# peterdavidfagan/mujoco_robot_environments

Measured on AMD Instinct MI355X. Metric: env steps/sec (whole node), RearrangementEnv batch=4096 at 1/2/4/8 MI355X, higher is better.
Workload: dtype f32

## Files before the change

### mujoco_robot_environments_amd/csrc/mre_api.cpp

```cpp
#include <hip/hip_runtime.h>

#include <cmath>
#include <cstdio>
#include <cstdlib>
#include <cstring>
#include <string>
#include <algorithm>
#include <vector>

#include "mre_env.h"
#include "mre_labels.h"
#include "mre_launch.h"
#include "mre_model.h"
#include "mre_records.h"

using namespace mre;

static thread_local std::string g_err;
int mre::fail(int code, const std::string& msg) {
  g_err = msg;
  return code;
}

extern "C" const char* mre_last_error(void) { return g_err.c_str(); }
// ... 29 lines not shown
  HIPCHK(hipMalloc(&e->sv_converged, N));
  HIPCHK(hipHostMalloc((void**)&e->h_launch_info, mre_env::RING * N * 16, hipHostMallocMapped | hipHostMallocCoherent));
  HIPCHK(hipHostGetDevicePointer((void**)&e->d_launch_info, e->h_launch_info, 0));
  memset(e->h_launch_info, 0xFF, mre_env::RING * N * 16);
  HIPCHK(hipHostMalloc((void**)&e->h_info_last, N * 16, hipHostMallocDefault));
  memset(e->h_info_last, 0xFF, N * 16);
  HIPCHK(hipHostMalloc((void**)&e->h_large_stage, mre_env::NSTAGE * N, hipHostMallocMapped | hipHostMallocCoherent));
  HIPCHK(hipHostGetDevicePointer((void**)&e->d_large_stage, e->h_large_stage, 0));
  memset(e->h_large_stage, 0, mre_env::NSTAGE * N);
  HIPCHK(hipMalloc(&e->d_pending, N));
  HIPCHK(hipMemsetAsync(e->d_pending, 0, N, e->stream));
  HIPCHK(hipMemsetAsync(e->d_large, 0, N, e->stream));
  e->h_large.assign(N, 0); e->h_rerun.assign(N, 0);
  { int rc = sched_create(e); if (rc) return rc; }
  if (const char* fb = getenv("MRE_NO_FALLBACK")) e->fallback = atoi(fb) == 0;
  if (const char* fl = getenv("MRE_FORCE_LARGE")) {
    if (atoi(fl) != 0) {
      e->h_large.assign(N, 1); e->n_large = num_envs;
      HIPCHK(hipMemsetAsync(e->d_large, 1, N, e->stream));
    }
  }
  HIPCHK(hipMemsetAsync(e->status, 0, N * 4, e->stream)); HIPCHK(hipMemsetAsync(e->stats, 0, N * 16, e->stream));
  HIPCHK(hipMemsetAsync(e->grip_closed, 0, N, e->stream)); HIPCHK(hipMemsetAsync(e->osc_target, 0, N * 64, e->stream));
  HIPCHK(hipMemsetAsync(e->sites, 0, N * 64, e->stream));
  std::vector<int> np(N, NPROP);
  std::vector<float> ps(N * NPROP * 3, 0.0155f);
  HIPCHK(hipMemcpy(e->nprops, np.data(), N * 4, hipMemcpyHostToDevice));
  HIPCHK(hipMemcpy(e->prop_size, ps.data(), ps.size() * 4, hipMemcpyHostToDevice));
  e->osc = OscConfig{350.f, 20.f, 500.f, 100.f, 200.f, 30.f, {0.f, -0.785f, 0.f, -2.356f, 0.f, 1.571f, 0.785f},
                     5e-3f, 68e-3f, 0};
// ... 574 lines not shown
  if (!e || !w) return fail(MRE_ERR_ARG, "null");
  DRAIN(e);
  return copy_out(e, w, e->qacc_ws, (size_t)e->N * NVP * 4);
}
extern "C" int mre_set_ctrl(mre_env* e, const float* ctrl) {
  if (!e || !ctrl) return fail(MRE_ERR_ARG, "null");
  DRAIN(e);
  return copy_in(e, e->ctrl, ctrl, (size_t)e->N * NU * 4);
}

static void fill_args(mre_env* e, StepArgs& a) {
  memset(&a, 0, sizeof(a));
  a.M = e->dM; a.N = e->N; a.seq_stride = e->N;
  a.qpos = e->qpos; a.qvel = e->qvel; a.qacc_ws = e->qacc_ws; a.ctrl = e->ctrl; a.qfine = e->qfine;
  a.nprops = e->nprops; a.prop_size = e->prop_size;
  a.control_steps = 1; a.mode = CTRL_HELD;
  a.osc = e->d_osc_env ? e->d_osc_env : e->d_osc; a.osc_stride = e->d_osc_env ? 1 : 0;
  a.osc_target = e->osc_target; a.grip_closed = e->grip_closed;
  a.sites = e->sites; a.status = e->status; a.stats = e->stats; a.nstep = e->nstep;
  a.env_order = e->use_order ? e->order : (e->have_auto_order ? e->auto_order : nullptr);
  a.trace = e->trace; a.trace_nenv = e->trace_nenv; a.trace_max = e->trace_max; a.trace_base = e->trace_pos;
}

extern "C" int mre_step(mre_env* e, int nsubsteps, unsigned flags) {
  if (!e || nsubsteps < 0) return fail(MRE_ERR_ARG, "mre_step: bad argument");
  StepArgs a;
  fill_args(e, a);
  a.nsteps = nsubsteps; a.flags = flags;
  if (nsubsteps > 0) a.sites = nullptr;
  int rc = launch_step(e, a);
  if (rc) return rc;
  if (e->trace) e->trace_pos += nsubsteps;
  return MRE_OK;
}

extern "C" int mre_rollout_ticks(mre_env* e, const float* ctrl_seq, int nticks, int control_steps, unsigned flags,
                                 int ticks_per_launch) {
  if (!e || !ctrl_seq || nticks < 0 || control_steps < 1) return fail(MRE_ERR_ARG, "mre_rollout: bad argument");
  if (!is_device_ptr(ctrl_seq)) return fail(MRE_ERR_ARG, "mre_rollout: ctrl_seq must be a device pointer");
  int per = (ticks_per_launch <= 0 || ticks_per_launch > nticks) ? nticks : ticks_per_launch;
  bool allow_queue = ticks_per_launch >= 2;
  if (ticks_per_launch <= 0 && policy::queue_fits(e->queue_ok, e->queue_waves, e->N) && nticks >= 2) {
    if (policy::window_wants_queue(nticks, e->queue_min_ticks, e->tick_tail_valid, e->tick_tail, e->queue_tail_min)) {
// ... 9 lines not shown
    const size_t n = (size_t)nticks * (size_t)e->N * NU;
    if (n > e->seq_cap) {
      DRAIN_PENDING(e);
      for (float*& p : e->seq_copy) { if (p) HIPCHK(hipFree(p)); p = nullptr; HIPCHK(hipMalloc(&p, n * 4)); }
      e->seq_cap = n;
    }
    float* dst = e->seq_copy[e->seq_calls++ % (unsigned)(mre_env::RING + 1)];
    HIPCHK(hipMemcpyAsync(dst, ctrl_seq, n * 4, hipMemcpyDeviceToDevice, e->stream));
    src = dst;
  }
  for (int t0 = 0; t0 < nticks || (nticks == 0 && t0 == 0); t0 += per) {
    const int nt = nticks - t0 < per ? nticks - t0 : per;
    StepArgs a;
    fill_args(e, a);
    a.nsteps = nt * control_steps; a.control_steps = control_steps; a.mode = CTRL_SEQ;
    a.ctrl_seq = src + (size_t)t0 * (size_t)e->N * NU; a.flags = flags;
    a.sites = nullptr;
    int rc = launch_step(e, a, false, true, allow_queue);
    if (rc) return rc;
    if (e->trace) e->trace_pos += a.nsteps;
    if (nticks == 0) break;
  }
  return MRE_OK;
}

extern "C" int mre_rollout(mre_env* e, const float* ctrl_seq, int nticks, int control_steps, unsigned flags) {
  return mre_rollout_ticks(e, ctrl_seq, nticks, control_steps, flags, 0);
}

extern "C" int mre_set_trace(mre_env* e, float* out, int nenv, int max_steps) {
  if (!e) return fail(MRE_ERR_ARG, "null handle");
// ... 152 lines not shown
    if (t0 + n < nticks) a.flags |= F_CONV_OPEN;
    int rc = launch_step(e, a, false, queue || !(converged_out != nullptr && chunk >= nticks), queue);
    if (rc) return rc;
    if (e->trace) e->trace_pos += a.nsteps;
    t0 += n;
  } while (t0 < nticks);
  if (converged_out) { DRAIN(e); return copy_out(e, converged_out, e->converged, (size_t)e->N); }
  return MRE_OK;
}

extern "C" int mre_osc_compute(mre_env* e, float* tau, float* grip) {
  if (!e) return fail(MRE_ERR_ARG, "null handle");
  DRAIN(e);
  StepArgs a;
  fill_args(e, a);
  a.nsteps = 0; a.control_steps = 1; a.mode = CTRL_OSC; a.flags = F_OSC_EVAL; a.trace = nullptr;
  HIPCHK(hipSetDevice(e->device));
  step_kernels(e->solver).step(&a, e->stream);
  HIPCHK(hipGetLastError());
  const size_t N = (size_t)e->N;
  std::vector<float> h(N * NU);
  int rc = copy_out(e, h.data(), e->ctrl, N * NU * 4);
  if (rc) return rc;
  std::vector<float> ht(N * 7), hg(N);
  for (size_t i = 0; i < N; i++) {
    for (int k = 0; k < 7; k++) ht[i * 7 + k] = h[i * NU + k];
    hg[i] = h[i * NU + 7];
  }
  if (tau) { rc = copy_out(e, tau, ht.data(), N * 7 * 4); if (rc) return rc; }
  if (grip) { rc = copy_out(e, grip, hg.data(), N * 4); if (rc) return rc; }
  return MRE_OK;
}

static int search_buffers(mre_env* e) {
  if (e->ps_attempts) return MRE_OK;
  const size_t N = (size_t)e->N;
  HIPCHK(hipMalloc(&e->ps_attempts, N * 4)); HIPCHK(hipMalloc(&e->ps_prop, N * 4));
  HIPCHK(hipMalloc(&e->ps_tick, N * 4)); HIPCHK(hipMalloc(&e->ps_which, N * 4));
  HIPCHK(hipMalloc(&e->ps_bounds, N * 6 * 8)); HIPCHK(hipMalloc(&e->ps_pose, N * 7 * 8));
  HIPCHK(hipMalloc(&e->ps_zones, N * NPROP * 4 * 8)); HIPCHK(hipMalloc(&e->ps_pick, N * 7 * 8));
  return MRE_OK;
}
static void fill_search(mre_env* e, SearchArgs& sa) {
  memset(&sa, 0, sizeof(sa));
  sa.M = e->dM; sa.N = e->N; sa.qpos = e->qpos; sa.qfine = e->qfine; sa.nprops = e->nprops; sa.prop_size = e->prop_size;
  sa.env_ids = e->d_env_ids; sa.env_id_offset = e->env_id_offset;
  sa.attempts = e->ps_attempts; sa.fixed_prop = -1;
}

static int detect_contacts(mre_env* e, const uint8_t* dmask, bool full = false, bool active_only = false) {
  const size_t N = (size_t)e->N, row = 1 + 3 * CONTACT_EXPORT;
  if (!e->contacts) HIPCHK(hipMalloc(&e->contacts, N * row * 4));
  if (full && !e->contacts_full) HIPCHK(hipMalloc(&e->contacts_full, N * CONTACT_EXPORT * 12 * 4));
  StepArgs a;
  fill_args(e, a);
  a.nsteps = 0; a.flags = F_DETECT | (active_only ? F_DETECT_ACTIVE : 0u); a.trace = nullptr; a.env_mask = dmask;
  a.contacts = e->contacts; a.contacts_full = full ? e->contacts_full : nullptr;
  a.sites = nullptr; a.geoms = nullptr;
  step_kernels(e->solver).step(&a, e->stream);
  HIPCHK(hipGetLastError());
  return MRE_OK;
}

extern "C" int mre_get_contacts(mre_env* e, int32_t* count, float* contacts) {
  if (!e || !count || !contacts) return fail(MRE_ERR_ARG, "mre_get_contacts: null");
  DRAIN(e);
  HIPCHK(hipSetDevice(e->device));
  int rc = detect_contacts(e, nullptr);
  if (rc) return rc;
  const size_t N = (size_t)e->N, row = 1 + 3 * CONTACT_EXPORT;
  std::vector<float> h(N * row);
// ... 97 lines not shown
      mre_launch_pose_search(&sa, e->stream);
      HIPCHK(hipGetLastError());
      if ((rc = copy_out(e, att.data(), e->ps_attempts, N * 4))) return rc;
      bool dropped = false;
      for (size_t i = 0; i < N; i++)
        if (todo[i] && p < np[i] && att[i] <= 0) { failed[i] = 1; todo[i] = 0; dropped = true; }
      if (dropped && (rc = copy_in(e, e->mask, todo.data(), N))) return rc;
    }
    HIPCHK(hipStreamSynchronize(e->stream));
    if (settle_steps <= 0) break;
    StepArgs a;
    fill_args(e, a);
    a.trace = nullptr;
    a.nsteps = (int)std::lround(2.0 / e->hM.opt_rec.timestep);
    if (a.nsteps < settle_steps) a.nsteps = settle_steps;
    a.flags = F_FREEZE_ROBOT | F_SETTLE_EXIT; a.env_mask = e->mask;
    a.settle_steps = e->settle_steps; a.min_settle_steps = settle_steps;
    const bool prof = e->profiling;
    e->profiling = false;
    rc = launch_step(e, a, true);
    e->profiling = prof;
    if (rc) return rc;
    if ((rc = copy_out(e, hs.data(), e->settle_steps, N * 4))) return rc;
    if (getenv("MRE_DEBUG_PLACE")) {
      int nt = 0, ns = 0;
      for (size_t i = 0; i < N; i++) if (todo[i]) { nt++; ns += hs[i] >= 0; }
      fprintf(stderr, "mre_place_props round %d: %d envs placed, %d settled\n", round, nt, ns);
    }
    int settled_now = 0;
    for (size_t i = 0; i < N; i++) {
      if (!todo[i]) continue;
// ... 159 lines not shown
```

### mujoco_robot_environments_amd/csrc/mre_collide.h

```cpp
#pragma once
#include "mre_math.h"

namespace mre {

constexpr int COLL_BUF = 48;
MRE_DEV float* cand_xyz(float* buf, int k) { return buf + 24 + 3 * k; }
MRE_DEV float& cand_dist(float* buf, int k) { return buf[3 * k + 2]; }

MRE_DEV float sel3(const float* v, int i) {
  const float w0 = i == 0 ? 1.f : 0.f, w1 = i == 1 ? 1.f : 0.f, w2 = i == 2 ? 1.f : 0.f;
  return w0 * v[0] + w1 * v[1] + w2 * v[2];
}
MRE_DEV void row3(float* o, const float (*m)[3], int i) {
  const float w0 = i == 0 ? 1.f : 0.f, w1 = i == 1 ? 1.f : 0.f, w2 = i == 2 ? 1.f : 0.f;
  o[0] = w0 * m[0][0] + w1 * m[1][0] + w2 * m[2][0];
  o[1] = w0 * m[0][1] + w1 * m[1][1] + w2 * m[2][1];
  o[2] = w0 * m[0][2] + w1 * m[1][2] + w2 * m[2][2];
}

MRE_DEV int clip_poly(float* p, float* q, int n, float sx, float sy) {
  float* src = p;
  float* dst = q;
  for (int e = 0; e < 4; e++) {
    const int ax = e >> 1;
// ... 10 lines not shown
      if (da <= 0 && nq < 8) { dst[3 * nq] = a0; dst[3 * nq + 1] = a1; dst[3 * nq + 2] = a2; nq++; }
      if ((da <= 0) != (db <= 0) && nq < 8) {
        const float t = da / (da - db);
        dst[3 * nq] = a0 + t * (b0 - a0); dst[3 * nq + 1] = a1 + t * (b1 - a1); dst[3 * nq + 2] = a2 + t * (b2 - a2);
        nq++;
      }
      a0 = b0; a1 = b1; a2 = b2;
    }
    n = nq;
    if (n == 0) return 0;
    float* t = src; src = dst; dst = t;
  }
  return n;
}

MRE_DEV int box_box(const float* p1, const float* R1, const float* s1, const float* p2,
                    const float* R2, const float* s2, float margin, float* normal, float* buf) {
  float* poly = buf;
  float* qbuf = buf + 24;
  float A[3][3], B[3][3], dv[3], Cm[3][3], aC[3][3];
#pragma unroll
  for (int i = 0; i < 3; i++)
#pragma unroll
    for (int k = 0; k < 3; k++) { A[i][k] = R1[3 * k + i]; B[i][k] = R2[3 * k + i]; }
  v3sub(dv, p2, p1);
#pragma unroll
  for (int i = 0; i < 3; i++)
#pragma unroll
    for (int j = 0; j < 3; j++) { Cm[i][j] = v3dot(A[i], B[j]); aC[i][j] = fabsf(Cm[i][j]); }
  float tA[3], tB[3];
#pragma unroll
  for (int i = 0; i < 3; i++) { tA[i] = v3dot(dv, A[i]); tB[i] = v3dot(dv, B[i]); }
// ... 92 lines not shown
    const float dd = fabsf(v3dot(nr, Ai[k]));
    if (dd > bestd) { bestd = dd; kk = k; }
  }
  const int ku = (kk + 1) % 3, kv = (kk + 2) % 3, au = (a + 1) % 3, av = (a + 2) % 3;
  float Aik[3], Aiu[3], Aiv[3], Aru[3], Arv[3];
  row3(Aik, Ai, kk); row3(Aiu, Ai, ku); row3(Aiv, Ai, kv);
  row3(Aru, Ar, au); row3(Arv, Ar, av);
  const float sik = sel3(siv3, kk), siu = sel3(siv3, ku), siv = sel3(siv3, kv);
  const float sra = sel3(srv3, a), sru = sel3(srv3, au), srv = sel3(srv3, av);
  const float isg = v3dot(nr, Aik) >= 0 ? -1.0f : 1.0f;
  float ci[3], cr[3];
  v3copy(ci, pi);
  v3addscl(ci, Aik, isg * sik);
  v3copy(cr, pr);
  v3addscl(cr, nr, sra);
#pragma unroll
  for (int v = 0; v < 4; v++) {
    const float su = (v == 0 || v == 3) ? 1.0f : -1.0f;
    const float sv = (v < 2) ? 1.0f : -1.0f;
    float w[3];
    v3copy(w, ci);
    v3addscl(w, Aiu, su * siu);
    v3addscl(w, Aiv, sv * siv);
    v3sub(w, w, cr);
    poly[3 * v] = v3dot(w, Aru);
    poly[3 * v + 1] = v3dot(w, Arv);
    poly[3 * v + 2] = v3dot(w, nr);
  }
  const int n = clip_poly(poly, qbuf, 4, sru, srv);
  int nc = 0;
  for (int v = 0; v < n; v++) {
    const float x = poly[3 * v], y = poly[3 * v + 1], dep = poly[3 * v + 2];
    if (dep > margin) continue;
    float* cx = cand_xyz(buf, nc);
    cx[0] = cr[0] + x * Aru[0] + y * Arv[0] + 0.5f * dep * nr[0];
    cx[1] = cr[1] + x * Aru[1] + y * Arv[1] + 0.5f * dep * nr[1];
    cx[2] = cr[2] + x * Aru[2] + y * Arv[2] + 0.5f * dep * nr[2];
    cand_dist(buf, nc) = dep;
    nc++;
  }
  return nc;
}

// ... 132 lines not shown
```

### mujoco_robot_environments_amd/csrc/mre_dev.h

```cpp
#pragma once
#include <stdint.h>

namespace mre {

constexpr int NB = 20;
constexpr int NRB = 16;
constexpr int GRIP_BODY0 = 8;
constexpr int NV = 39;
constexpr int NRV = 15;
constexpr int NQ = 43;
constexpr int NQP = 44;
constexpr int TRACE_W = 88;
constexpr int TRACE_QVEL = 48;
constexpr int NVP = 40;
constexpr int NU = 8;
constexpr int QFINE = 32;
constexpr int QFINE_ROW = 96;
constexpr int QFINE_CUBE_Q = 32;
constexpr int QFINE_CUBE_V = 60;
static_assert(QFINE_CUBE_Q + 7 * 4 == QFINE_CUBE_V && QFINE_CUBE_V + 6 * 4 <= QFINE_ROW, "qfine row layout");
constexpr int NPROP = 4;
constexpr int NG = 20;
constexpr int PROP_GEOM0 = 12;
constexpr int NPAIR = 128;
// ... 138 lines not shown
  MEntryRec m_rec[NMR];
  RowRec row_rec[NROWREC];
  EqRec eq_rec[NEQ];
  SiteRec site_rec[NSITE];
  OptRec opt_rec;
};

struct OscConfig {
  float kp_pos, kd_pos, kp_ori, kd_ori, kp_null, kd_null;
  float null_q[7];
  float pos_thresh, ori_thresh;
  int pinv_always;
};

enum StepFlags : unsigned { F_NO_CONSTRAINTS = 1u, F_FREEZE_ROBOT = 2u, F_CONV_CONTINUE = 4u, F_CONV_OPEN = 8u,
                            F_OSC_EVAL = 16u, F_DETECT = 32u, F_SETTLE_EXIT = 64u, F_DETECT_ACTIVE = 128u };
enum CtrlMode : int { CTRL_HELD = 0, CTRL_SEQ = 1, CTRL_OSC = 2 };

struct StepArgs {
  const DevModel* M;
  int N;
  float* qpos;
  float* qvel;
  float* qacc_ws;
  float* qfine;
  float* ctrl;
  const float* ctrl_seq;
  int seq_stride;
  const int* nprops;
  const float* prop_size;
  int nsteps, control_steps, mode;
// ... 53 lines not shown
  unsigned long long seed;
  const int* prop;
  int fixed_prop;
  const double* bounds;
  double shared_bounds[6];
  const int* tick_base;
  long long tick0;
  int max_attempts;
  int yaw_mode;
  double fixed_quat[4];
  float max_dist;
  int commit;
  float* qfine;
  double* pose;
  int* attempts;
};

constexpr int DYN_W = 128;
constexpr int DYN_JAC = 0, DYN_MASS = 42, DYN_BIAS = 91, DYN_POS = 98, DYN_QUAT = 101, DYN_QPOS = 105, DYN_QVEL = 112,
              DYN_PAD = 119;
struct DynArgs {
  const DevModel* M;
  int N;
  const float* qpos;
  const float* qvel;
  const float* qfine;
  const int* nprops;
  const float* prop_size;
  int site;
  float* out;
// ... 38 lines not shown
```

### mujoco_robot_environments_amd/csrc/mre_env.h

```cpp
#pragma once
#include <hip/hip_runtime.h>

#include <string>
#include <utility>
#include <vector>

#include "../../include/mre.h"
#include "mre_dev.h"
#include "mre_policy.h"

#define HIPCHK(x)                                                                       \
  do {                                                                                  \
    hipError_t e_ = (x);                                                                \
    if (e_ != hipSuccess)                                                               \
      return mre::fail(MRE_ERR_HIP, std::string(#x) + ": " + hipGetErrorString(e_));    \
  } while (0)

struct mre_env {
  int N = 0, device = 0;
  hipStream_t stream = nullptr;
  mre::DevModel* dM = nullptr;
  mre::DevModel hM;
  int solver = MRE_SOLVER_PGS;
  float *qpos = nullptr, *qvel = nullptr, *qacc_ws = nullptr, *ctrl = nullptr;
// ... 17 lines not shown
  uint8_t* prop_rgb = nullptr;
  float geom_rgb[mre::NG][3];
  float* trace = nullptr;
  int trace_nenv = 0, trace_max = 0, trace_pos = 0;
  long long env_id_offset = 0;
  std::vector<long long> env_ids;
  int* order = nullptr;
  bool use_order = false;
  int* auto_order = nullptr;
  int* h_auto_order = nullptr;
  bool have_auto_order = false;
  bool profiling = false;
  std::vector<std::pair<hipEvent_t, hipEvent_t>> events;
  size_t events_used = 0;
  bool fallback = true;
  bool large_only = false;
  bool compact_only = false;
  hipStream_t stream2 = nullptr;
  hipEvent_t ev_fork = nullptr, ev_join = nullptr, ev_order = nullptr;
  uint8_t *d_large = nullptr, *mask_r = nullptr;
  float *sv_qpos = nullptr, *sv_qvel = nullptr, *sv_qacc_ws = nullptr, *sv_ctrl = nullptr, *sv_qfine = nullptr;
  uint32_t* sv_status = nullptr;
  uint8_t* sv_converged = nullptr;
  float* contacts = nullptr;
  float* contacts_full = nullptr;
  int* settle_steps = nullptr;
  int* h_launch_info = nullptr;
  int* d_launch_info = nullptr;
  int* h_info_last = nullptr;
  uint8_t* d_pending = nullptr;
// ... 86 lines not shown
```

### mujoco_robot_environments_amd/csrc/mre_kernels.hip

```cpp
#include <hip/hip_runtime.h>

#include "mre_dev.h"
#include "mre_math.h"
#include "mre_collide.h"

namespace mre {
using ModelP = MRE_MODEL_PTR(DevModel);
#if defined(MRE_PHASE_STAMPS) && MRE_PHASE_STAMPS >= 4
__shared__ unsigned long long dbg_acc[4];
#endif

struct OscSm {
  float J[6][7], M[7][7], MiJt[7][6], Li[6][6], Lam[6][6], V[6][6], Jbar[7][6];
  float ep[3], eo[3], F[6], LF[6], tn[7], Jbt[6], xd[6], w[6];
};

struct alignas(8) Blk {
  uint16_t row0;
  uint8_t type, nrows;
  uint8_t rslot;
  uint8_t pa, pb;
  uint8_t primary : 4;
  uint8_t bslot : 4;
};
// ... 1382 lines not shown
    crb_mass_matrix(M, s, l);
    MRE_SYNC();
#ifndef MRE_NEWTON
    factor_robot_regs(s.qM, s.qLD, s.qLDinv);
#endif
    MRE_STAMP(15);
    MRE_STAMP(0);

    velocity_stage(M, s, l);
    MRE_SYNC();
    finger_bias(M, s, l);
    MRE_STAMP(1);
    const bool constrained = (a.flags & F_NO_CONSTRAINTS) == 0;
    if (constrained) {

      collide(M, s, l, false);
      MRE_STAMP(2);
      assemble_constraints(M, s, l);
#ifdef MRE_NEWTON
      nw_build_lists(s, l);
#else
      solve_robot_rows(s, l);
      assemble_blocks(M, s, l);
#endif
      MRE_STAMP(3);
      hw_ncon = max(hw_ncon, s.ncon); hw_nefc = max(hw_nefc, s.nefc);
      hw_nrrow = max(hw_nrrow, s.nrrow); hw_npp = max(hw_npp, s.npp);
    }

    if (a.mode == CTRL_SEQ && (step % a.control_steps) == 0) {
      const int tick = step / a.control_steps;
// ... 85 lines not shown
    else a.nstep[env] += steps_done;
  }
  if (a.nsteps == 0 && (a.flags & F_OSC_EVAL) != 0 && a.mode == CTRL_OSC) {
    position_stage(M, s, l);
    gripper_local(M, s, l);
    crb_mass_matrix(M, s, l);
    MRE_SYNC();
    velocity_stage(M, s, l);
    MRE_SYNC();
    osc_compute(M, s, osc, oscp, s.osc_tgt, l);
    if (l == 0) s.ctrl[NU - 1] = grip_cmd;
    MRE_SYNC();
  }
  if (a.nsteps == 0 && (a.flags & F_DETECT) != 0 && a.contacts != nullptr) {
    position_stage(M, s, l);
    collide(M, s, l, (a.flags & F_DETECT_ACTIVE) == 0);
    float* o = a.contacts + (size_t)env * (1 + 3 * CONTACT_EXPORT);
    const int n = s.ncon < CONTACT_EXPORT ? s.ncon : CONTACT_EXPORT;
    if (l == 0) o[0] = s.overflow ? -(float)s.ncon : (float)s.ncon;
    if (l < n) {
      const int pr = s.con_pair[l];
      o[1 + 3 * l] = (float)M->pair_g1[pr]; o[2 + 3 * l] = (float)M->pair_g2[pr]; o[3 + 3 * l] = s.con_dist[l];
      if (a.contacts_full != nullptr) {
        float* f = a.contacts_full + ((size_t)env * CONTACT_EXPORT + l) * 12;
        for (int k = 0; k < 3; k++) f[k] = s.con_pos[l][k];
        for (int k = 0; k < 9; k++) f[3 + k] = s.con_frame[l][k];
      }
    }
    MRE_SYNC();
    if (l == 0) s.overflow = 0;
  }
// ... 237 lines not shown
      float xq[4] = {(float)pose[3], (float)pose[4], (float)pose[5], (float)pose[6]};
      qnormalize(xq);
      for (int k = 0; k < 3; k++) s.xpos[body][k] = (float)pose[k];
      for (int k = 0; k < 4; k++) s.xquat[body][k] = xq[k];
      q2mat(s.xmat[body], xq);
    }
    MRE_SYNC();
    bool hit = false;
    if (pr >= 0) {
      const int g1 = M->pair_g1[pr], g2 = M->pair_g2[pr];
      float p1[3], R1[9], s1[3], rb1, p2[3], R2[9], s2[3], rb2, normal[3] = {0.f, 0.f, 1.f}, df[3];
      geom_pose(M, s, g1, p1, R1, s1, &rb1);
      geom_pose(M, s, g2, p2, R2, s2, &rb2);
      const float inc = M->pair_margin[pr];
      int n = 0;
      v3sub(df, p2, p1);
      if (M->geom_type[g1] == 0) {
        float nn[3] = {R1[2], R1[5], R1[8]};
        if (v3dot(df, nn) - rb2 <= inc) n = plane_box(p1, R1, p2, R2, s2, inc, normal, buf);
      } else {
        const float r = rb1 + rb2 + inc;
        if (v3dot(df, df) <= r * r) n = box_box(p1, R1, s1, p2, R2, s2, inc, normal, buf);
      }
      for (int c = 0; c < n; c++) {
        const float d = cand_dist(buf, c);
        if (d < inc && d <= a.max_dist) hit = true;
      }
    }
    const bool any = __ballot(hit) != 0ull;
    MRE_SYNC();
    if (!any) { used = att + 1; break; }
  }
  if (l == 0) {
    if (a.attempts != nullptr) a.attempts[env] = used;
    if (used > 0) {
      if (a.pose != nullptr) for (int k = 0; k < 7; k++) a.pose[(size_t)env * 7 + k] = pose[k];
      if (a.commit) {
        float* q = a.qpos + (size_t)env * NQP + NRV + 7 * p;
        for (int k = 0; k < 7; k++) q[k] = (float)pose[k];
        if (a.qfine != nullptr) {
          float* ql = a.qfine + (size_t)env * QFINE_ROW;
// ... 207 lines not shown
```

### mujoco_robot_environments_amd/csrc/mre_math.h

```cpp
#pragma once
#include <hip/hip_runtime.h>

#define MRE_DEV __device__ __forceinline__
#if defined(MRE_PHASE_STAMPS) && MRE_PHASE_STAMPS >= 4
#define MRE_DBG_T0() unsigned long long dbg_t_ = __builtin_amdgcn_s_memtime()
#define MRE_DBG_STAMP(SET, K)                                                      \
  do {                                                                             \
    const unsigned long long n_ = __builtin_amdgcn_s_memtime();                    \
    if (MRE_PHASE_STAMPS == (SET) && threadIdx.x == 0) dbg_acc[K] += n_ - dbg_t_;  \
    dbg_t_ = n_;                                                                   \
  } while (0)
#else
#define MRE_DBG_T0() do {} while (0)
#define MRE_DBG_STAMP(SET, K) do {} while (0)
#endif
#define MRE_PHASE_FN __device__ __attribute__((noinline))
#define MRE_SYNC()                                        \
  do {                                                    \
    __builtin_amdgcn_fence(__ATOMIC_ACQ_REL, "wavefront"); \
    __builtin_amdgcn_wave_barrier();                      \
  } while (0)
#if defined(__HIP_DEVICE_COMPILE__)
#define MRE_MODEL_PTR(T) const T __attribute__((address_space(1)))*
#else
#define MRE_MODEL_PTR(T) const T*
#endif

namespace mre {

constexpr float kMinVal = 1e-15f;

MRE_DEV void keep_live(float x) { asm volatile("" ::"v"(x)); }
MRE_DEV void keep_live(int x) { asm volatile("" ::"v"(x)); }

MRE_DEV void v3copy(float* r, const float* a) { r[0] = a[0]; r[1] = a[1]; r[2] = a[2]; }
MRE_DEV void v3zero(float* r) { r[0] = r[1] = r[2] = 0.f; }
MRE_DEV void v3add(float* r, const float* a, const float* b) {
  r[0] = a[0] + b[0]; r[1] = a[1] + b[1]; r[2] = a[2] + b[2];
}
MRE_DEV void v3sub(float* r, const float* a, const float* b) {
  r[0] = a[0] - b[0]; r[1] = a[1] - b[1]; r[2] = a[2] - b[2];
}
MRE_DEV float v3dot(const float* a, const float* b) { return a[0] * b[0] + a[1] * b[1] + a[2] * b[2]; }
MRE_DEV void v3cross(float* r, const float* a, const float* b) {
  float x = a[1] * b[2] - a[2] * b[1], y = a[2] * b[0] - a[0] * b[2], z = a[0] * b[1] - a[1] * b[0];
  r[0] = x; r[1] = y; r[2] = z;
}
MRE_DEV void v3addscl(float* r, const float* a, float s) { r[0] += a[0] * s; r[1] += a[1] * s; r[2] += a[2] * s; }
// ... 90 lines not shown
  v3cross(r, vel, v);
  v3cross(a, vel, v + 3);
  v3cross(b, vel + 3, v);
  v3add(r + 3, a, b);
}
MRE_DEV void cross_force(float* r, const float* vel, const float* f) {
  float a[3], b[3];
  v3cross(a, vel, f);
  v3cross(b, vel + 3, f + 3);
  v3add(r, a, b);
  v3cross(r + 3, vel, f + 3);
}
MRE_DEV float dot6(const float* a, const float* b) {
  return a[0] * b[0] + a[1] * b[1] + a[2] * b[2] + a[3] * b[3] + a[4] * b[4] + a[5] * b[5];
}
template <int CTRL, int ROW_MASK>
MRE_DEV float dpp_add(float v) {
  const int t = __builtin_amdgcn_update_dpp(0, __builtin_bit_cast(int, v), CTRL, ROW_MASK, 0xF, false);
  return v + __builtin_bit_cast(float, t);
}
MRE_DEV float wave_sum(float v) {
  v = dpp_add<0xB1, 0xF>(v);
  v = dpp_add<0x4E, 0xF>(v);
  v = dpp_add<0x141, 0xF>(v);
  v = dpp_add<0x140, 0xF>(v);
  v = dpp_add<0x142, 0xA>(v);
  v = dpp_add<0x143, 0xC>(v);
  return __builtin_bit_cast(float, __builtin_amdgcn_readlane(__builtin_bit_cast(int, v), 63));
}
MRE_DEV void wave_sum3(float& a, float& b, float& c) {
// ... 25 lines not shown
}
template <int CTRL, int ROW_MASK>
MRE_DEV float dpp_max(float v) {
  const int t = __builtin_amdgcn_update_dpp(0, __builtin_bit_cast(int, v), CTRL, ROW_MASK, 0xF, false);
  return fmaxf(v, __builtin_bit_cast(float, t));
}
MRE_DEV float wave_max(float v) {
  v = dpp_max<0xB1, 0xF>(v);
  v = dpp_max<0x4E, 0xF>(v);
  v = dpp_max<0x141, 0xF>(v);
  v = dpp_max<0x140, 0xF>(v);
  v = dpp_max<0x142, 0xA>(v);
  v = dpp_max<0x143, 0xC>(v);
  return __builtin_bit_cast(float, __builtin_amdgcn_readlane(__builtin_bit_cast(int, v), 63));
}
MRE_DEV float clampf(float x, float lo, float hi) { return x < lo ? lo : (x > hi ? hi : x); }

MRE_DEV double rcp64(double x) {
  double r = __builtin_amdgcn_rcp(x);
  r = r * (2.0 - x * r);
  return r * (2.0 - x * r);
}
MRE_DEV double rsq64(double x) {
  double y = __builtin_amdgcn_rsq(x);
  y = y * (1.5 - 0.5 * x * y * y);
  return y * (1.5 - 0.5 * x * y * y);
}


}
```

### mujoco_robot_environments_amd/csrc/mre_solver.h

```cpp
#pragma once

namespace mre {

constexpr int HDR_NONE = 0xFF;
constexpr int BLK_NONE = 0x7F;
constexpr int SCHED_NONE = 0xFF;
constexpr int TAB_OFF = MAXBLK * 5;
constexpr int TAB_ZEROS = 48;
static_assert(TAB_BYTES == 8 * (TAB_OFF + 1) + 4 * TAB_ZEROS, "operand table size");

#ifndef MRE_NEWTON
MRE_DEV void build_schedule(ModelP M, Sm& s);
#endif
MRE_DEV constexpr int cube_pair_bit(int p, int q) {
  const int a = p < q ? p : q, b = p < q ? q : p;
  return a == 0 ? b - 1 : (a == 1 ? b + 1 : 5);
}

MRE_DEV float prop_invM(const Sm& s, int p, int k) {
  return 1.0f / ((k < 3) ? s.prop_mass[p] : s.prop_inertia[p][k - 3]);
}

MRE_DEV void geom_pose(ModelP M, const Sm& s, int g, float* p, float* R, float* size,
                       float* rbound) {
// ... 10 lines not shown
  } else {
    v3copy(size, M->geom_size[g]);
    *rbound = M->geom_rbound[g];
  }
}

MRE_DEV void geom_center(ModelP M, const Sm& s, int g, float* p, float* rbound) {
  const int b = M->geom_body[g];
  float tmp[3];
  m3mulv(tmp, s.xmat[b], M->geom_pos[g]);
  v3add(p, s.xpos[b], tmp);
  const int pid = M->geom_propid[g];
  *rbound = pid >= 0 ? v3norm(s.prop_size[pid]) : M->geom_rbound[g];
}

MRE_PHASE_FN void collide(ModelP M, Sm& s, int l, bool detect) {
  static_assert(offsetof(Sm, hdr) + sizeof(((Sm*)0)->hdr) - offsetof(Sm, JpA) >= sizeof(float) * 64 * COLL_BUF,
                "clip buffers do not fit");
  static_assert(NPAIR <= 256 && sizeof(((Sm*)0)->iscr) >= NPAIR, "survivor list: one byte per pair");
  MRE_DBG_T0();
  float* buf = &s.JpA[0][0] + l * COLL_BUF;
  uint8_t* list = reinterpret_cast<uint8_t*>(s.iscr);
  const unsigned long long lt = (1ull << l) - 1ull;
  int nsurv = 0;
  for (int pass = 0; pass < NPAIR / 64; pass++) {
    const int pr = l + 64 * pass;
    const auto* R = &M->pair_rec[pr];
    const int g1 = R->g1, b1 = R->b1, b2 = R->b2, pid1 = R->pid1, pid2 = R->pid2, type1 = R->type1;
    const float lp1[3] = {R->pos1[0], R->pos1[1], R->pos1[2]}, lp2[3] = {R->pos2[0], R->pos2[1], R->pos2[2]};
    const float mrb1 = R->rb1, mrb2 = R->rb2, margin = R->margin, gap = R->gap;
    const float lq1[4] = {R->quat1[0], R->quat1[1], R->quat1[2], R->quat1[3]};
    bool live = false;
    if (g1 >= 0 && (pid1 < 0 || pid1 < s.nprops) && (pid2 < 0 || pid2 < s.nprops)) {
      const float inc = detect ? margin : margin - gap;
      float p1[3], p2[3], df[3], tmp[3];
      m3mulv(tmp, s.xmat[b1], lp1); v3add(p1, s.xpos[b1], tmp);
// ... 6 lines not shown
        q2mat(R1, q);
        const float nn[3] = {R1[2], R1[5], R1[8]};
        live = v3dot(df, nn) - rb2 <= inc;
      } else {
        const float r = rb1 + rb2 + inc;
        live = v3dot(df, df) <= r * r;
      }
    }
    const unsigned long long m = __ballot(live);
    if (live) list[nsurv + __popcll(m & lt)] = (uint8_t)pr;
    nsurv += __popcll(m);
  }
  if (l == 0) s.ncon = 0;
  MRE_SYNC();
  MRE_DBG_STAMP(6, 0);
  int base = 0;
  for (int c0 = 0; c0 < nsurv; c0 += 64) {
    const int pr = (c0 + l < nsurv) ? list[c0 + l] : -1;
    float normal[3] = {0.f, 0.f, 1.f};
    int n = 0;
    if (pr >= 0) {
      const auto* R = &M->pair_rec[pr];
      const int b1 = R->b1, b2 = R->b2, pid1 = R->pid1, pid2 = R->pid2, type1 = R->type1;
      const float lp1[3] = {R->pos1[0], R->pos1[1], R->pos1[2]}, lp2[3] = {R->pos2[0], R->pos2[1], R->pos2[2]};
      const float lq1[4] = {R->quat1[0], R->quat1[1], R->quat1[2], R->quat1[3]};
      const float lq2[4] = {R->quat2[0], R->quat2[1], R->quat2[2], R->quat2[3]};
      const float ms1[3] = {R->size1[0], R->size1[1], R->size1[2]}, ms2[3] = {R->size2[0], R->size2[1], R->size2[2]};
      const float margin = R->margin, gap = R->gap;
      float p1[3], R1[9], s1[3], p2[3], R2[9], s2[3], tmp[3], q[4];
      m3mulv(tmp, s.xmat[b1], lp1); v3add(p1, s.xpos[b1], tmp);
      qmul(q, s.xquat[b1], lq1); q2mat(R1, q);
      m3mulv(tmp, s.xmat[b2], lp2); v3add(p2, s.xpos[b2], tmp);
      qmul(q, s.xquat[b2], lq2); q2mat(R2, q);
      if (pid1 >= 0) v3copy(s1, s.prop_size[pid1]); else v3copy(s1, ms1);
      if (pid2 >= 0) v3copy(s2, s.prop_size[pid2]); else v3copy(s2, ms2);
      const float inc = detect ? margin : margin - gap;
      MRE_DBG_STAMP(6, 1);
      if ((R->single >> 8) == 2) n = cyl_box(p1, R1, s1, p2, R2, s2[0], s2[2], inc, normal, buf);
      else if (type1 == 0) n = plane_box(p1, R1, p2, R2, s2, inc, normal, buf);
      else n = box_box(p1, R1, s1, p2, R2, s2, inc, normal, buf);
      MRE_DBG_STAMP(6, 2);
      int m = 0;
      for (int c = 0; c < n; c++)
        if (cand_dist(buf, c) < inc) {
          if (m != c) {
            for (int k = 0; k < 3; k++) cand_xyz(buf, m)[k] = cand_xyz(buf, c)[k];
            cand_dist(buf, m) = cand_dist(buf, c);
          }
          m++;
        }
      n = m;
    }
    const bool single = pr >= 0 && n > 1 && (M->pair_rec[pr].single & 0xFF) != 0;
    const int ncand = n;
    if (single) n = 1;
    int off = base, tot = base;
    for (int bit = 0; bit < 4; bit++) {
      const unsigned long long m = __ballot((n >> bit) & 1);
      off += __popcll(m & lt) << bit;
      tot += __popcll(m) << bit;
    }
    if (l == 0) {
      s.ncon = tot < NCON_MAX ? tot : NCON_MAX;
      if (tot > NCON_MAX) s.overflow = 1;
    }
    if (single) {
      const float incw = M->pair_rec[pr].margin - M->pair_rec[pr].gap;
      float wsum = 0.f, px = 0.f, py = 0.f, pz = 0.f, dmin = cand_dist(buf, 0);
      int best = 0;
      for (int c = 0; c < ncand; c++) {
        const float dc = cand_dist(buf, c);
        if (dc < dmin) { dmin = dc; best = c; }
        const float w = incw - dc;
        if (w > 0.f) { wsum += w; px += w * cand_xyz(buf, c)[0]; py += w * cand_xyz(buf, c)[1]; pz += w * cand_xyz(buf, c)[2]; }
      }
      if (wsum > 0.f) { const float iw = 1.0f / wsum; px *= iw; py *= iw; pz *= iw; }
      else { px = cand_xyz(buf, best)[0]; py = cand_xyz(buf, best)[1]; pz = cand_xyz(buf, best)[2]; }
      cand_xyz(buf, 0)[0] = px; cand_xyz(buf, 0)[1] = py; cand_xyz(buf, 0)[2] = pz;
      cand_dist(buf, 0) = dmin;
    }
    if (n > 0) {
      float f[9];
      v3copy(f, normal);
      make_frame(f);
      for (int c = 0; c < n; c++) {
        const int id = off + c;
        if (id >= NCON_MAX) break;
        const float cx0 = cand_xyz(buf, c)[0], cx1 = cand_xyz(buf, c)[1], cx2 = cand_xyz(buf, c)[2];
        s.con_pos[id][0] = cx0; s.con_pos[id][1] = cx1; s.con_pos[id][2] = cx2;
        for (int k = 0; k < 9; k++) s.con_frame[id][k] = f[k];
        s.con_dist[id] = cand_dist(buf, c);
        s.con_pair[id] = (uint8_t)pr;
      }
    }
    MRE_SYNC();
    MRE_DBG_STAMP(6, 3);
    if (tot > NCON_MAX) break;
    base = tot;
  }
}

MRE_DEV float impedance(const float* solimp, float pos, float margin) {
  const float dmin = clampf(solimp[0], 0.0001f, 0.9999f), dmax = clampf(solimp[1], 0.0001f, 0.9999f);
  const float width = fmaxf(solimp[2], kMinVal), mid = clampf(solimp[3], 0.0001f, 0.9999f);
  const float power = fmaxf(solimp[4], 1.0f);
  if (dmin == dmax) return 0.5f * (dmin + dmax);
  const float x = fabsf((pos - margin) / width);
  if (x >= 1.0f) return dmax;
  if (x <= 0.0f) return dmin;
  float y;
  if (power == 1.0f) y = x;
  else if (power == 2.0f) {
    y = (x <= mid) ? x * x / mid : 1.0f - (1.0f - x) * (1.0f - x) / (1.0f - mid);
// ... 855 lines not shown
```

Baseline: 24.58 million.

## Keep unclipped box-box face contacts in registers instead of LDS clip buffer

Adds a fast path in box_box: when all four incident-face vertices already lie inside the reference face rectangle, contact candidates are computed directly into a register struct, skipping the polygon clip and the per-lane shared-memory candidate buffer. Downstream filtering, single-contact averaging and contact emission get matching register-based branches. Collide is split into broad and narrow phase functions, and an env-var flag can force the old clipping path. This adds code size and register pressure, and the extra branches may diverge within a wavefront.

```diff
diff --git a/mujoco_robot_environments_amd/csrc/mre_api.cpp b/mujoco_robot_environments_amd/csrc/mre_api.cpp
--- a/mujoco_robot_environments_amd/csrc/mre_api.cpp
+++ b/mujoco_robot_environments_amd/csrc/mre_api.cpp
@@ -67,6 +67,7 @@
   e->h_large.assign(N, 0); e->h_rerun.assign(N, 0);
   { int rc = sched_create(e); if (rc) return rc; }
   if (const char* fb = getenv("MRE_NO_FALLBACK")) e->fallback = atoi(fb) == 0;
+  if (const char* ng = getenv("MRE_NARROW_GENERIC")) e->base_flags = atoi(ng) != 0 ? F_CLIP_ALWAYS : 0u;
   if (const char* fl = getenv("MRE_FORCE_LARGE")) {
     if (atoi(fl) != 0) {
       e->h_large.assign(N, 1); e->n_large = num_envs;
@@ -671,7 +672,7 @@
   a.M = e->dM; a.N = e->N; a.seq_stride = e->N;
   a.qpos = e->qpos; a.qvel = e->qvel; a.qacc_ws = e->qacc_ws; a.ctrl = e->ctrl; a.qfine = e->qfine;
   a.nprops = e->nprops; a.prop_size = e->prop_size;
-  a.control_steps = 1; a.mode = CTRL_HELD;
+  a.control_steps = 1; a.mode = CTRL_HELD; a.flags = e->base_flags;
   a.osc = e->d_osc_env ? e->d_osc_env : e->d_osc; a.osc_stride = e->d_osc_env ? 1 : 0;
   a.osc_target = e->osc_target; a.grip_closed = e->grip_closed;
   a.sites = e->sites; a.status = e->status; a.stats = e->stats; a.nstep = e->nstep;
@@ -683,7 +684,7 @@
   if (!e || nsubsteps < 0) return fail(MRE_ERR_ARG, "mre_step: bad argument");
   StepArgs a;
   fill_args(e, a);
-  a.nsteps = nsubsteps; a.flags = flags;
+  a.nsteps = nsubsteps; a.flags |= flags;
   if (nsubsteps > 0) a.sites = nullptr;
   int rc = launch_step(e, a);
   if (rc) return rc;
@@ -723,7 +724,7 @@
     StepArgs a;
     fill_args(e, a);
     a.nsteps = nt * control_steps; a.control_steps = control_steps; a.mode = CTRL_SEQ;
-    a.ctrl_seq = src + (size_t)t0 * (size_t)e->N * NU; a.flags = flags;
+    a.ctrl_seq = src + (size_t)t0 * (size_t)e->N * NU; a.flags |= flags;
     a.sites = nullptr;
     int rc = launch_step(e, a, false, true, allow_queue);
     if (rc) return rc;
@@ -906,7 +907,7 @@
   DRAIN(e);
   StepArgs a;
   fill_args(e, a);
-  a.nsteps = 0; a.control_steps = 1; a.mode = CTRL_OSC; a.flags = F_OSC_EVAL; a.trace = nullptr;
+  a.nsteps = 0; a.control_steps = 1; a.mode = CTRL_OSC; a.flags |= F_OSC_EVAL; a.trace = nullptr;
   HIPCHK(hipSetDevice(e->device));
   step_kernels(e->solver).step(&a, e->stream);
   HIPCHK(hipGetLastError());
@@ -937,7 +938,7 @@
   memset(&sa, 0, sizeof(sa));
   sa.M = e->dM; sa.N = e->N; sa.qpos = e->qpos; sa.qfine = e->qfine; sa.nprops = e->nprops; sa.prop_size = e->prop_size;
   sa.env_ids = e->d_env_ids; sa.env_id_offset = e->env_id_offset;
-  sa.attempts = e->ps_attempts; sa.fixed_prop = -1;
+  sa.attempts = e->ps_attempts; sa.fixed_prop = -1; sa.flags = e->base_flags;
 }
 
 static int detect_contacts(mre_env* e, const uint8_t* dmask, bool full = false, bool active_only = false) {
@@ -946,7 +947,7 @@
   if (full && !e->contacts_full) HIPCHK(hipMalloc(&e->contacts_full, N * CONTACT_EXPORT * 12 * 4));
   StepArgs a;
   fill_args(e, a);
-  a.nsteps = 0; a.flags = F_DETECT | (active_only ? F_DETECT_ACTIVE : 0u); a.trace = nullptr; a.env_mask = dmask;
+  a.nsteps = 0; a.flags |= F_DETECT | (active_only ? F_DETECT_ACTIVE : 0u); a.trace = nullptr; a.env_mask = dmask;
   a.contacts = e->contacts; a.contacts_full = full ? e->contacts_full : nullptr;
   a.sites = nullptr; a.geoms = nullptr;
   step_kernels(e->solver).step(&a, e->stream);
@@ -1074,7 +1075,7 @@
     a.trace = nullptr;
     a.nsteps = (int)std::lround(2.0 / e->hM.opt_rec.timestep);
     if (a.nsteps < settle_steps) a.nsteps = settle_steps;
-    a.flags = F_FREEZE_ROBOT | F_SETTLE_EXIT; a.env_mask = e->mask;
+    a.flags |= F_FREEZE_ROBOT | F_SETTLE_EXIT; a.env_mask = e->mask;
     a.settle_steps = e->settle_steps; a.min_settle_steps = settle_steps;
     const bool prof = e->profiling;
     e->profiling = false;
diff --git a/mujoco_robot_environments_amd/csrc/mre_collide.h b/mujoco_robot_environments_amd/csrc/mre_collide.h
--- a/mujoco_robot_environments_amd/csrc/mre_collide.h
+++ b/mujoco_robot_environments_amd/csrc/mre_collide.h
@@ -6,6 +6,10 @@
 constexpr int COLL_BUF = 48;
 MRE_DEV float* cand_xyz(float* buf, int k) { return buf + 24 + 3 * k; }
 MRE_DEV float& cand_dist(float* buf, int k) { return buf[3 * k + 2]; }
+
+struct FaceCand { float x[4], y[4], z[4], d[4]; };
+constexpr unsigned FACE_IN_REGS = 16u;
+constexpr unsigned FACE_BRANCH = 32u;
 
 MRE_DEV float sel3(const float* v, int i) {
   const float w0 = i == 0 ? 1.f : 0.f, w1 = i == 1 ? 1.f : 0.f, w2 = i == 2 ? 1.f : 0.f;
@@ -48,8 +52,12 @@
   return n;
 }
 
+MRE_DEV bool clip_keeps(float sg, float coord, float lim) { return sg * coord - lim <= 0; }
+
 MRE_DEV int box_box(const float* p1, const float* R1, const float* s1, const float* p2,
-                    const float* R2, const float* s2, float margin, float* normal, float* buf) {
+                    const float* R2, const float* s2, float margin, float* normal, float* buf,
+                    bool clip_always, FaceCand& rc, unsigned& rmask) {
+  rmask = 0u;
   float* poly = buf;
   float* qbuf = buf + 24;
   float A[3][3], B[3][3], dv[3], Cm[3][3], aC[3][3];
@@ -172,6 +180,7 @@
   v3addscl(ci, Aik, isg * sik);
   v3copy(cr, pr);
   v3addscl(cr, nr, sra);
+  float vx[4], vy[4], vd[4];
 #pragma unroll
   for (int v = 0; v < 4; v++) {
     const float su = (v == 0 || v == 3) ? 1.0f : -1.0f;
@@ -181,10 +190,34 @@
     v3addscl(w, Aiu, su * siu);
     v3addscl(w, Aiv, sv * siv);
     v3sub(w, w, cr);
-    poly[3 * v] = v3dot(w, Aru);
-    poly[3 * v + 1] = v3dot(w, Arv);
-    poly[3 * v + 2] = v3dot(w, nr);
-  }
+    vx[v] = v3dot(w, Aru);
+    vy[v] = v3dot(w, Arv);
+    vd[v] = v3dot(w, nr);
+  }
+#if defined(MRE_PHASE_STAMPS)
+  rmask = FACE_BRANCH;
+#endif
+  bool inside = !clip_always;
+#pragma unroll
+  for (int v = 0; v < 4; v++)
+    inside = inside && clip_keeps(1.0f, vx[v], sru) && clip_keeps(-1.0f, vx[v], sru) &&
+             clip_keeps(1.0f, vy[v], srv) && clip_keeps(-1.0f, vy[v], srv);
+  if (inside) {
+    rmask |= FACE_IN_REGS;
+    int nc = 0;
+#pragma unroll
+    for (int v = 0; v < 4; v++) {
+      const float x = vx[v], y = vy[v], dep = vd[v];
+      rc.x[v] = cr[0] + x * Aru[0] + y * Arv[0] + 0.5f * dep * nr[0];
+      rc.y[v] = cr[1] + x * Aru[1] + y * Arv[1] + 0.5f * dep * nr[1];
+      rc.z[v] = cr[2] + x * Aru[2] + y * Arv[2] + 0.5f * dep * nr[2];
+      rc.d[v] = dep;
+      if (!(dep > margin)) { rmask |= 1u << v; nc++; }
+    }
+    return nc;
+  }
+#pragma unroll
+  for (int v = 0; v < 4; v++) { poly[3 * v] = vx[v]; poly[3 * v + 1] = vy[v]; poly[3 * v + 2] = vd[v]; }
   const int n = clip_poly(poly, qbuf, 4, sru, srv);
   int nc = 0;
   for (int v = 0; v < n; v++) {
diff --git a/mujoco_robot_environments_amd/csrc/mre_dev.h b/mujoco_robot_environments_amd/csrc/mre_dev.h
--- a/mujoco_robot_environments_amd/csrc/mre_dev.h
+++ b/mujoco_robot_environments_amd/csrc/mre_dev.h
@@ -176,7 +176,8 @@
 };
 
 enum StepFlags : unsigned { F_NO_CONSTRAINTS = 1u, F_FREEZE_ROBOT = 2u, F_CONV_CONTINUE = 4u, F_CONV_OPEN = 8u,
-                            F_OSC_EVAL = 16u, F_DETECT = 32u, F_SETTLE_EXIT = 64u, F_DETECT_ACTIVE = 128u };
+                            F_OSC_EVAL = 16u, F_DETECT = 32u, F_SETTLE_EXIT = 64u, F_DETECT_ACTIVE = 128u,
+                            F_CLIP_ALWAYS = 256u };
 enum CtrlMode : int { CTRL_HELD = 0, CTRL_SEQ = 1, CTRL_OSC = 2 };
 
 struct StepArgs {
@@ -260,6 +261,7 @@
   float* qfine;
   double* pose;
   int* attempts;
+  unsigned flags;
 };
 
 constexpr int DYN_W = 128;
diff --git a/mujoco_robot_environments_amd/csrc/mre_env.h b/mujoco_robot_environments_amd/csrc/mre_env.h
--- a/mujoco_robot_environments_amd/csrc/mre_env.h
+++ b/mujoco_robot_environments_amd/csrc/mre_env.h
@@ -55,6 +55,7 @@
   std::vector<std::pair<hipEvent_t, hipEvent_t>> events;
   size_t events_used = 0;
   bool fallback = true;
+  unsigned base_flags = 0;
   bool large_only = false;
   bool compact_only = false;
   hipStream_t stream2 = nullptr;
diff --git a/mujoco_robot_environments_amd/csrc/mre_kernels.hip b/mujoco_robot_environments_amd/csrc/mre_kernels.hip
--- a/mujoco_robot_environments_amd/csrc/mre_kernels.hip
+++ b/mujoco_robot_environments_amd/csrc/mre_kernels.hip
@@ -1420,7 +1420,7 @@
     const bool constrained = (a.flags & F_NO_CONSTRAINTS) == 0;
     if (constrained) {
 
-      collide(M, s, l, false);
+      collide(M, s, l, false, (a.flags & F_CLIP_ALWAYS) != 0);
       MRE_STAMP(2);
       assemble_constraints(M, s, l);
 #ifdef MRE_NEWTON
@@ -1536,7 +1536,7 @@
   }
   if (a.nsteps == 0 && (a.flags & F_DETECT) != 0 && a.contacts != nullptr) {
     position_stage(M, s, l);
-    collide(M, s, l, (a.flags & F_DETECT_ACTIVE) == 0);
+    collide(M, s, l, (a.flags & F_DETECT_ACTIVE) == 0, (a.flags & F_CLIP_ALWAYS) != 0);
     float* o = a.contacts + (size_t)env * (1 + 3 * CONTACT_EXPORT);
     const int n = s.ncon < CONTACT_EXPORT ? s.ncon : CONTACT_EXPORT;
     if (l == 0) o[0] = s.overflow ? -(float)s.ncon : (float)s.ncon;
@@ -1804,17 +1804,25 @@
       geom_pose(M, s, g2, p2, R2, s2, &rb2);
       const float inc = M->pair_margin[pr];
       int n = 0;
+      FaceCand rc;
+      unsigned rm = 0u;
       v3sub(df, p2, p1);
       if (M->geom_type[g1] == 0) {
         float nn[3] = {R1[2], R1[5], R1[8]};
         if (v3dot(df, nn) - rb2 <= inc) n = plane_box(p1, R1, p2, R2, s2, inc, normal, buf);
       } else {
         const float r = rb1 + rb2 + inc;
-        if (v3dot(df, df) <= r * r) n = box_box(p1, R1, s1, p2, R2, s2, inc, normal, buf);
+        if (v3dot(df, df) <= r * r) n = box_box(p1, R1, s1, p2, R2, s2, inc, normal, buf, (a.flags & F_CLIP_ALWAYS) != 0, rc, rm);
       }
-      for (int c = 0; c < n; c++) {
-        const float d = cand_dist(buf, c);
-        if (d < inc && d <= a.max_dist) hit = true;
+      if (rm & FACE_IN_REGS) {
+#pragma unroll
+        for (int v = 0; v < 4; v++)
+          if (((rm >> v) & 1u) != 0u && rc.d[v] < inc && rc.d[v] <= a.max_dist) hit = true;
+      } else {
+        for (int c = 0; c < n; c++) {
+          const float d = cand_dist(buf, c);
+          if (d < inc && d <= a.max_dist) hit = true;
+        }
       }
     }
     const bool any = __ballot(hit) != 0ull;
diff --git a/mujoco_robot_environments_amd/csrc/mre_math.h b/mujoco_robot_environments_amd/csrc/mre_math.h
--- a/mujoco_robot_environments_amd/csrc/mre_math.h
+++ b/mujoco_robot_environments_amd/csrc/mre_math.h
@@ -1,7 +1,10 @@
 #pragma once
+#ifndef MRE_DEV
 #include <hip/hip_runtime.h>
-
 #define MRE_DEV __device__ __forceinline__
+#else
+#define MRE_PER_LANE_ONLY
+#endif
 #if defined(MRE_PHASE_STAMPS) && MRE_PHASE_STAMPS >= 4
 #define MRE_DBG_T0() unsigned long long dbg_t_ = __builtin_amdgcn_s_memtime()
 #define MRE_DBG_STAMP(SET, K)                                                      \
@@ -30,8 +33,10 @@
 
 constexpr float kMinVal = 1e-15f;
 
+#ifndef MRE_PER_LANE_ONLY
 MRE_DEV void keep_live(float x) { asm volatile("" ::"v"(x)); }
 MRE_DEV void keep_live(int x) { asm volatile("" ::"v"(x)); }
+#endif
 
 MRE_DEV void v3copy(float* r, const float* a) { r[0] = a[0]; r[1] = a[1]; r[2] = a[2]; }
 MRE_DEV void v3zero(float* r) { r[0] = r[1] = r[2] = 0.f; }
@@ -152,6 +157,7 @@
 MRE_DEV float dot6(const float* a, const float* b) {
   return a[0] * b[0] + a[1] * b[1] + a[2] * b[2] + a[3] * b[3] + a[4] * b[4] + a[5] * b[5];
 }
+#ifndef MRE_PER_LANE_ONLY
 template <int CTRL, int ROW_MASK>
 MRE_DEV float dpp_add(float v) {
   const int t = __builtin_amdgcn_update_dpp(0, __builtin_bit_cast(int, v), CTRL, ROW_MASK, 0xF, false);
@@ -207,8 +213,10 @@
   v = dpp_max<0x143, 0xC>(v);
   return __builtin_bit_cast(float, __builtin_amdgcn_readlane(__builtin_bit_cast(int, v), 63));
 }
+#endif
 MRE_DEV float clampf(float x, float lo, float hi) { return x < lo ? lo : (x > hi ? hi : x); }
 
+#ifndef MRE_PER_LANE_ONLY
 MRE_DEV double rcp64(double x) {
   double r = __builtin_amdgcn_rcp(x);
   r = r * (2.0 - x * r);
@@ -219,6 +227,6 @@
   y = y * (1.5 - 0.5 * x * y * y);
   return y * (1.5 - 0.5 * x * y * y);
 }
-
-
-}
+#endif
+
+}
diff --git a/mujoco_robot_environments_amd/csrc/mre_solver.h b/mujoco_robot_environments_amd/csrc/mre_solver.h
--- a/mujoco_robot_environments_amd/csrc/mre_solver.h
+++ b/mujoco_robot_environments_amd/csrc/mre_solver.h
@@ -48,12 +48,11 @@
   *rbound = pid >= 0 ? v3norm(s.prop_size[pid]) : M->geom_rbound[g];
 }
 
-MRE_PHASE_FN void collide(ModelP M, Sm& s, int l, bool detect) {
+MRE_PHASE_FN int collide_broad(ModelP M, Sm& s, int l, bool detect) {
   static_assert(offsetof(Sm, hdr) + sizeof(((Sm*)0)->hdr) - offsetof(Sm, JpA) >= sizeof(float) * 64 * COLL_BUF,
                 "clip buffers do not fit");
   static_assert(NPAIR <= 256 && sizeof(((Sm*)0)->iscr) >= NPAIR, "survivor list: one byte per pair");
   MRE_DBG_T0();
-  float* buf = &s.JpA[0][0] + l * COLL_BUF;
   uint8_t* list = reinterpret_cast<uint8_t*>(s.iscr);
   const unsigned long long lt = (1ull << l) - 1ull;
   int nsurv = 0;
@@ -90,11 +89,19 @@
   if (l == 0) s.ncon = 0;
   MRE_SYNC();
   MRE_DBG_STAMP(6, 0);
-  int base = 0;
-  for (int c0 = 0; c0 < nsurv; c0 += 64) {
+  return nsurv;
+}
+MRE_PHASE_FN int collide_narrow(ModelP M, Sm& s, int l, bool detect, bool clip_always, int c0, int nsurv, int base) {
+  MRE_DBG_T0();
+  float* buf = &s.JpA[0][0] + l * COLL_BUF;
+  const uint8_t* list = reinterpret_cast<const uint8_t*>(s.iscr);
+  const unsigned long long lt = (1ull << l) - 1ull;
+  {
     const int pr = (c0 + l < nsurv) ? list[c0 + l] : -1;
     float normal[3] = {0.f, 0.f, 1.f};
     int n = 0;
+    FaceCand rc;
+    unsigned rm = 0u;
     if (pr >= 0) {
       const auto* R = &M->pair_rec[pr];
       const int b1 = R->b1, b2 = R->b2, pid1 = R->pid1, pid2 = R->pid2, type1 = R->type1;
@@ -114,19 +121,37 @@
       MRE_DBG_STAMP(6, 1);
       if ((R->single >> 8) == 2) n = cyl_box(p1, R1, s1, p2, R2, s2[0], s2[2], inc, normal, buf);
       else if (type1 == 0) n = plane_box(p1, R1, p2, R2, s2, inc, normal, buf);
-      else n = box_box(p1, R1, s1, p2, R2, s2, inc, normal, buf);
+      else n = box_box(p1, R1, s1, p2, R2, s2, inc, normal, buf, clip_always, rc, rm);
       MRE_DBG_STAMP(6, 2);
       int m = 0;
-      for (int c = 0; c < n; c++)
-        if (cand_dist(buf, c) < inc) {
-          if (m != c) {
-            for (int k = 0; k < 3; k++) cand_xyz(buf, m)[k] = cand_xyz(buf, c)[k];
-            cand_dist(buf, m) = cand_dist(buf, c);
+      if (rm & FACE_IN_REGS) {
+#pragma unroll
+        for (int v = 0; v < 4; v++) {
+          if (((rm >> v) & 1u) != 0u && rc.d[v] < inc) m++;
+          else rm &= ~(1u << v);
+        }
+      } else {
+        for (int c = 0; c < n; c++)
+          if (cand_dist(buf, c) < inc) {
+            if (m != c) {
+              for (int k = 0; k < 3; k++) cand_xyz(buf, m)[k] = cand_xyz(buf, c)[k];
+              cand_dist(buf, m) = cand_dist(buf, c);
+            }
+            m++;
           }
-          m++;
-        }
+      }
       n = m;
     }
+#if defined(MRE_PHASE_STAMPS) && MRE_PHASE_STAMPS == 8
+    {
+      const bool tbl = pr >= 0 && (M->pair_rec[pr].g1 == 1);
+      const unsigned long long fb = __ballot((rm & FACE_BRANCH) != 0u), fr = __ballot((rm & FACE_IN_REGS) != 0u), tb = __ballot(tbl);
+      if (l == 0) {
+        dbg_acc[0] += (unsigned long long)__popcll(fb) << 4; dbg_acc[1] += (unsigned long long)__popcll(fr) << 4;
+        dbg_acc[2] += (unsigned long long)__popcll(fb & tb) << 4; dbg_acc[3] += (unsigned long long)__popcll(fr & tb) << 4;
+      }
+    }
+#endif
     const bool single = pr >= 0 && n > 1 && (M->pair_rec[pr].single & 0xFF) != 0;
     const int ncand = n;
     if (single) n = 1;
@@ -142,37 +167,75 @@
     }
     if (single) {
       const float incw = M->pair_rec[pr].margin - M->pair_rec[pr].gap;
-      float wsum = 0.f, px = 0.f, py = 0.f, pz = 0.f, dmin = cand_dist(buf, 0);
-      int best = 0;
-      for (int c = 0; c < ncand; c++) {
-        const float dc = cand_dist(buf, c);
-        if (dc < dmin) { dmin = dc; best = c; }
-        const float w = incw - dc;
-        if (w > 0.f) { wsum += w; px += w * cand_xyz(buf, c)[0]; py += w * cand_xyz(buf, c)[1]; pz += w * cand_xyz(buf, c)[2]; }
-      }
-      if (wsum > 0.f) { const float iw = 1.0f / wsum; px *= iw; py *= iw; pz *= iw; }
-      else { px = cand_xyz(buf, best)[0]; py = cand_xyz(buf, best)[1]; pz = cand_xyz(buf, best)[2]; }
-      cand_xyz(buf, 0)[0] = px; cand_xyz(buf, 0)[1] = py; cand_xyz(buf, 0)[2] = pz;
-      cand_dist(buf, 0) = dmin;
+      if (rm & FACE_IN_REGS) {
+        float wsum = 0.f, px = 0.f, py = 0.f, pz = 0.f, dmin = 0.f, bx = 0.f, by = 0.f, bz = 0.f;
+        bool first = true;
+#pragma unroll
+        for (int v = 0; v < 4; v++)
+          if (((rm >> v) & 1u) != 0u) {
+            const float dc = rc.d[v];
+            if (first || dc < dmin) { dmin = dc; bx = rc.x[v]; by = rc.y[v]; bz = rc.z[v]; }
+            first = false;
+            const float w = incw - dc;
+            if (w > 0.f) { wsum += w; px += w * rc.x[v]; py += w * rc.y[v]; pz += w * rc.z[v]; }
+          }
+        if (wsum > 0.f) { const float iw = 1.0f / wsum; px *= iw; py *= iw; pz *= iw; }
+        else { px = bx; py = by; pz = bz; }
+        rc.x[0] = px; rc.y[0] = py; rc.z[0] = pz; rc.d[0] = dmin;
+        rm = FACE_IN_REGS | 1u;
+      } else {
+        float wsum = 0.f, px = 0.f, py = 0.f, pz = 0.f, dmin = cand_dist(buf, 0);
+        int best = 0;
+        for (int c = 0; c < ncand; c++) {
+          const float dc = cand_dist(buf, c);
+          if (dc < dmin) { dmin = dc; best = c; }
+          const float w = incw - dc;
+          if (w > 0.f) { wsum += w; px += w * cand_xyz(buf, c)[0]; py += w * cand_xyz(buf, c)[1]; pz += w * cand_xyz(buf, c)[2]; }
+        }
+        if (wsum > 0.f) { const float iw = 1.0f / wsum; px *= iw; py *= iw; pz *= iw; }
+        else { px = cand_xyz(buf, best)[0]; py = cand_xyz(buf, best)[1]; pz = cand_xyz(buf, best)[2]; }
+        cand_xyz(buf, 0)[0] = px; cand_xyz(buf, 0)[1] = py; cand_xyz(buf, 0)[2] = pz;
+        cand_dist(buf, 0) = dmin;
+      }
     }
     if (n > 0) {
       float f[9];
       v3copy(f, normal);
       make_frame(f);
-      for (int c = 0; c < n; c++) {
-        const int id = off + c;
-        if (id >= NCON_MAX) break;
-        const float cx0 = cand_xyz(buf, c)[0], cx1 = cand_xyz(buf, c)[1], cx2 = cand_xyz(buf, c)[2];
-        s.con_pos[id][0] = cx0; s.con_pos[id][1] = cx1; s.con_pos[id][2] = cx2;
-        for (int k = 0; k < 9; k++) s.con_frame[id][k] = f[k];
-        s.con_dist[id] = cand_dist(buf, c);
-        s.con_pair[id] = (uint8_t)pr;
+      if (rm & FACE_IN_REGS) {
+        int id = off;
+#pragma unroll
+        for (int v = 0; v < 4; v++)
+          if (((rm >> v) & 1u) != 0u && id < NCON_MAX) {
+            s.con_pos[id][0] = rc.x[v]; s.con_pos[id][1] = rc.y[v]; s.con_pos[id][2] = rc.z[v];
+            for (int k = 0; k < 9; k++) s.con_frame[id][k] = f[k];
+            s.con_dist[id] = rc.d[v];
+            s.con_pair[id] = (uint8_t)pr;
+            id++;
+          }
+      } else {
+        for (int c = 0; c < n; c++) {
+          const int id = off + c;
+          if (id >= NCON_MAX) break;
+          const float cx0 = cand_xyz(buf, c)[0], cx1 = cand_xyz(buf, c)[1], cx2 = cand_xyz(buf, c)[2];
+          s.con_pos[id][0] = cx0; s.con_pos[id][1] = cx1; s.con_pos[id][2] = cx2;
+          for (int k = 0; k < 9; k++) s.con_frame[id][k] = f[k];
+          s.con_dist[id] = cand_dist(buf, c);
+          s.con_pair[id] = (uint8_t)pr;
+        }
       }
     }
     MRE_SYNC();
     MRE_DBG_STAMP(6, 3);
-    if (tot > NCON_MAX) break;
-    base = tot;
+    return tot;
+  }
+}
+MRE_DEV void collide(ModelP M, Sm& s, int l, bool detect, bool clip_always) {
+  const int nsurv = collide_broad(M, s, l, detect);
+  int base = 0;
+  for (int c0 = 0; c0 < nsurv; c0 += 64) {
+    base = collide_narrow(M, s, l, detect, clip_always, c0, nsurv, base);
+    if (base > NCON_MAX) break;
   }
 }
 
```

Measured after the change: 25.29 million (median of 6 runs). 2.9% higher.
